# amansanghvi/Thesis

Measured on AMD Instinct MI355X. Metric: particle-updates/sec (particles x scans/s) @1081 beams, higher is better.
Workload: dtype int8 map cells (lattice log-odds), f64 poses/weights; 1 GPU; BASELINE configs[2]: room16 synthetic, 4096 particles/GPU, 1081 beams, 0.05 m grid, K=30 samples, both matcher stages, resample every step; particles_per_gpu=4096, beams=1081, parallelism=particles sharded x1

## Files before the change

thesis_amd/csrc/kernels_resample.hip:

```cpp
#include <limits.h>

#include "rbpf_internal.h"

namespace rbpf {

static const int PLAN_THREADS = 1024;

__device__ __forceinline__ dd dd_two_prod(double a, double b) {
    double p = a * b;
    double e = __fma_rn(a, b, -p);
    return {p, e};
}
__device__ __forceinline__ dd dd_mul_d(dd a, double b) {
    dd p = dd_two_prod(a.hi, b);
    double lo = p.lo + a.lo * b;
    double hi = p.hi + lo;
    return {hi, lo - (hi - p.hi)};
}
__device__ __forceinline__ dd dd_sub(dd a, dd b) { return dd_add(a, dd{-b.hi, -b.lo}); }
__device__ __forceinline__ dd dd_div_d(dd a, double b) {
    double q1 = a.hi / b;
    dd r = dd_sub(a, dd_two_prod(q1, b));
    double q2 = (r.hi + r.lo) / b;
    double hi = q1 + q2;
// ... 359 lines not shown
    if (threadIdx.x == 0) *n_pending = 0;
}

__global__ void export_weights_kernel(int P, const double* __restrict__ w, const int32_t* __restrict__ gid,
                                      double* __restrict__ out, int n_global, const uint8_t* __restrict__ bad) {
    int p = blockIdx.x * blockDim.x + threadIdx.x;
    if (p < P && gid[p] >= 0 && gid[p] < n_global) out[gid[p]] = w[p];
    if (p < P && bad && bad[p]) out[n_global] = 1.0;
}

__device__ void sources_to_T_stage(int P, const int32_t* __restrict__ idx, int32_t* __restrict__ T, int32_t* __restrict__ did) {
    __shared__ int s_buf[PLAN_THREADS];
    const int tid = threadIdx.x, nt = PLAN_THREADS;
    const int chunk = (P + nt - 1) / nt;
    const int i0 = min(tid * chunk, P), i1 = min(i0 + chunk, P);
    for (int i = i0; i < i1; ++i) T[i] = 0;
    __syncthreads();
    for (int j = i0; j < i1; ++j) if (idx[j] >= 0) atomicAdd(&T[idx[j]], 1);
    __syncthreads();
    int sum = 0;
    for (int i = i0; i < i1; ++i) sum += T[i];
    int total;
    int run = block_exclusive_scan_1024(sum, s_buf, tid, total);
    for (int i = i0; i < i1; ++i) { run += T[i]; T[i] = run; }
    if (tid == 0) *did = 1;
}

__global__ void gather_meta_kernel(DevView v, const int32_t* __restrict__ local_idx, int n, int32_t* __restrict__ out) {
    const int LL = v.L * v.L;
    int q = blockIdx.x * blockDim.x + threadIdx.x;
    if (q >= n * LL) return;
    const int i = q / LL, pos = q % LL;
    const int t = v.tile_tab[(size_t)v.slot[local_idx[i]] * LL + pos];
    int32_t* o = out + (size_t)q * 5;
    o[0] = t;
    for (int k = 0; k < 4; ++k) o[1 + k] = t >= 0 ? v.tile_bbox[4 * t + k] : 0;
}

struct PackJob { int32_t particle, tile, x0, x1, ya, yb; long long off; };

__global__ __launch_bounds__(BLOCK) void pack_kernel(DevView v, const PackJob* __restrict__ jobs, unsigned char* __restrict__ buf) {
    const PackJob j = jobs[blockIdx.x];
    const int tid = threadIdx.x;
    unsigned char* dst = buf + j.off;
    if (j.tile < 0) {
        if (tid < 13) {
            const int p = j.particle;
            double val = tid == 0 ? v.px[p] : tid == 1 ? v.py[p] : tid == 2 ? v.pth[p]
                       : tid < 12 ? v.cov[(size_t)(tid - 3) * v.P + p] : v.weight[p];
            reinterpret_cast<double*>(dst)[tid] = val;
        }
        return;
    }
    const size_t cells = (size_t)v.dim * v.dim;
    const int8_t* src = v.pool + (size_t)j.tile * cells;
    const int per_row = (j.yb - j.ya) / 16, rows = j.x1 - j.x0 + 1;
    for (int q = tid; q < rows * per_row; q += BLOCK) {
        const int x = j.x0 + q / per_row, y = j.ya + (q % per_row) * 16;
        reinterpret_cast<uint4*>(dst)[q] = *reinterpret_cast<const uint4*>(src + (size_t)x * v.dim + y);
    }
    uint32_t* docc = reinterpret_cast<uint32_t*>(dst + (size_t)rows * per_row * 16);
    const uint32_t* socc = v.occ + ((size_t)j.tile * v.dim + j.x0) * v.ow;
    for (int q = tid; q < rows * v.ow; q += BLOCK) docc[q] = socc[q];
}

struct UnpackJob { int32_t particle, pos, has, x0, x1, ya, yb, pad; long long off; };

__global__ __launch_bounds__(BLOCK) void unpack_kernel(DevView v, const UnpackJob* __restrict__ jobs, const unsigned char* __restrict__ buf,
                                                       int32_t* pending_free, int32_t* n_pending) {
    __shared__ int s_tile;
    const UnpackJob j = jobs[blockIdx.x];
    const int tid = threadIdx.x, LL = v.L * v.L;
    if (j.pos < 0) {
        if (tid < 13) {
            const double val = reinterpret_cast<const double*>(buf + j.off)[tid];
            const int p = j.particle;
            if (tid == 0) v.px[p] = val; else if (tid == 1) v.py[p] = val; else if (tid == 2) v.pth[p] = val;
            else if (tid < 12) v.cov[(size_t)(tid - 3) * v.P + p] = val; else v.weight[p] = 1.0;
        }
        return;
    }
    const int slot = v.slot[j.particle];
    int td = v.tile_tab[(size_t)slot * LL + j.pos];
    const size_t cells = (size_t)v.dim * v.dim;
    if (!j.has) {
        if (td < 0) return;
        int db[4];
        for (int k = 0; k < 4; ++k) db[k] = v.tile_bbox[4 * td + k];
        if (db[0] <= db[1] && db[2] <= db[3]) {
            copy_rows<BLOCK>(v.pool + (size_t)td * cells, nullptr, v.dim, db[0], db[1], db[2], db[3], tid);
            copy_occ_rows<BLOCK>(v.occ + (size_t)td * v.dim * v.ow, nullptr, v.ow, db[0], db[1], db[2], db[3], tid);
        }
        if (tid == 0) {
            v.tile_bbox[4 * td + 0] = INT_MAX; v.tile_bbox[4 * td + 1] = -1; v.tile_bbox[4 * td + 2] = INT_MAX; v.tile_bbox[4 * td + 3] = -1;
            v.tile_tab[(size_t)slot * LL + j.pos] = -1;
            pending_free[atomicAdd(n_pending, 1)] = td;
        }
        return;
    }
    if (td < 0) {
        if (tid == 0) {
            int idx = atomicSub(v.free_top, 1) - 1;
            if (idx < 0) { atomicAdd(v.free_top, 1); atomicCAS(v.err, 0, RBPF_ENOMEM); s_tile = -1; }
            else { s_tile = v.free_stack[idx]; v.tile_tab[(size_t)slot * LL + j.pos] = s_tile; }
        }
        __syncthreads();
        td = s_tile;
        if (td < 0) return;
    } else {
        int db[4];
        for (int k = 0; k < 4; ++k) db[k] = v.tile_bbox[4 * td + k];
        if (db[0] <= db[1] && db[2] <= db[3]) {
            copy_rows<BLOCK>(v.pool + (size_t)td * cells, nullptr, v.dim, db[0], db[1], db[2], db[3], tid);
            copy_occ_rows<BLOCK>(v.occ + (size_t)td * v.dim * v.ow, nullptr, v.ow, db[0], db[1], db[2], db[3], tid);
        }
        __syncthreads();
    }
    if (j.x0 <= j.x1) {
        const unsigned char* src = buf + j.off;
        int8_t* dst = v.pool + (size_t)td * cells;
        const int per_row = (j.yb - j.ya) / 16, rows = j.x1 - j.x0 + 1;
        for (int q = tid; q < rows * per_row; q += BLOCK) {
            const int x = j.x0 + q / per_row, y = j.ya + (q % per_row) * 16;
            *reinterpret_cast<uint4*>(dst + (size_t)x * v.dim + y) = reinterpret_cast<const uint4*>(src)[q];
        }
        const uint32_t* socc = reinterpret_cast<const uint32_t*>(src + (size_t)rows * per_row * 16);
        uint32_t* docc = v.occ + ((size_t)td * v.dim + j.x0) * v.ow;
        for (int q = tid; q < rows * v.ow; q += BLOCK) docc[q] = socc[q];
    }
    if (tid == 0) { v.tile_bbox[4 * td + 0] = j.x0; v.tile_bbox[4 * td + 1] = j.x1; v.tile_bbox[4 * td + 2] = j.ya; v.tile_bbox[4 * td + 3] = j.yb - 1; }
}

__global__ __launch_bounds__(PLAN_THREADS) void resample_plan_kernel(ResampleArgs a, PhaseArgs ph) {
    if (ph.phase == 1 ? !plan_phase_verdict(a.P, ph) : plan_phase_idle(ph)) return;
    resample_plan_stage(a);
}
__global__ void resample_expand_kernel(int P, const int32_t* __restrict__ T, int32_t* __restrict__ idx, PhaseArgs ph) {
    if (plan_phase_idle(ph)) return;
    const int j = blockIdx.x * blockDim.x + threadIdx.x;
    if (j < P) resample_expand_one(P, T, idx, j);
}
__global__ __launch_bounds__(PLAN_THREADS) void resample_pair_kernel(PairArgs a, PhaseArgs ph) {
    if (plan_phase_idle(ph)) {
        if (ph.phase == 1) plan_keep_stage(a.P, a.T, false, ph);
        return;
    }
    resample_pair_stage(a);
    if (ph.phase == 1) { __syncthreads(); plan_keep_stage(a.P, a.T, ph.leave_out && *a.did, ph); }
}
__global__ __launch_bounds__(PLAN_THREADS) void sources_to_T_kernel(int P, const int32_t* __restrict__ idx, int32_t* __restrict__ T,
                                                                     int32_t* __restrict__ did) { sources_to_T_stage(P, idx, T, did); }

enum { RS_PLAN = 1, RS_SRC2T = 2, RS_EXPAND = 4, RS_PAIR = 8, RS_GATHER = 16 };
static const int RS_FUSE_MAX = 4096;
static const int RS_GATHER_FUSE_MAX = 1024;
struct FusedArgs { int stages; ResampleArgs ra; int32_t* idx; PairArgs pa; GatherArgs ga; PhaseArgs ph; };
__global__ __launch_bounds__(PLAN_THREADS) void resample_fused_kernel(FusedArgs f) {
    extern __shared__ __align__(16) int32_t s_dyn[];
    int32_t* const s_T = s_dyn; int32_t* const s_idx = s_dyn + RS_FUSE_MAX;
    const int tid = threadIdx.x, P = f.ra.P;
#ifdef RBPF_STAMPS
    long long st[6]; st[0] = clock64();
#define RSTAMP(k) st[k] = clock64()
#else
#define RSTAMP(k) do { } while (0)
#endif
    if (f.ph.phase == 1) {
        if (!plan_phase_verdict(P, f.ph)) { plan_keep_stage(P, f.ra.T, false, f.ph); return; }
    } else if (plan_phase_idle(f.ph)) return;
    if (f.stages & RS_PLAN) { resample_plan_stage(f.ra); __syncthreads(); }
    RSTAMP(1);
    if (f.stages & RS_SRC2T) { sources_to_T_stage(P, f.idx, f.ra.T, f.ra.did); __syncthreads(); }
    for (int j = tid; j < P; j += PLAN_THREADS) s_T[j] = f.ra.T[j];
    __syncthreads();
    if (f.stages & RS_EXPAND) { for (int j = tid; j < P; j += PLAN_THREADS) { resample_expand_one(P, s_T, s_idx, j); f.idx[j] = s_idx[j]; } }
    else for (int j = tid; j < P; j += PLAN_THREADS) s_idx[j] = f.idx[j];
    __syncthreads();
    RSTAMP(2);
    if (f.stages & RS_PAIR) { PairArgs pa = f.pa; pa.T = s_T; pa.idx = s_idx; resample_pair_stage(pa); __syncthreads(); }
    if (f.ph.phase == 1) plan_keep_stage(P, s_T, f.ph.leave_out && *f.ra.did, f.ph);
    RSTAMP(3);
    if (f.stages & RS_GATHER) { GatherArgs ga = f.ga; ga.T = s_T; ga.idx = s_idx; for (int j = tid; j < ga.P; j += PLAN_THREADS) resample_gather_one(ga, j); }
    RSTAMP(4);
#ifdef RBPF_STAMPS
    if (tid == 0) printf("resample_fused: plan %lld expand %lld pair %lld gather %lld cycles\n", st[1] - st[0], st[2] - st[1], st[3] - st[2], st[4] - st[3]);
#endif
}

static void launch_resample_fused(const FusedArgs& f, hipStream_t s) {
    const size_t lds = 2 * RS_FUSE_MAX * sizeof(int32_t);
    static size_t lds_set[MAX_DEVICES] = {};
    ensure_dynamic_lds(reinterpret_cast<const void*>(resample_fused_kernel), lds, lds_set);
    hipLaunchKernelGGL(resample_fused_kernel, dim3(1), dim3(PLAN_THREADS), lds, s, f);
}

void launch_export_weights(const DevView& v, double* d_out, int n_global, const uint8_t* d_bad, hipStream_t s) {
    (void)hipMemsetAsync(d_out, 0, (size_t)(n_global + (d_bad ? 1 : 0)) * 8, s);
    hipLaunchKernelGGL(export_weights_kernel, dim3((v.P + 255) / 256), dim3(256), 0, s, v.P, v.weight, v.global_id, d_out, n_global, d_bad);
}
void launch_gather_meta(const DevView& v, const int32_t* d_local, int n, int32_t* d_out, hipStream_t s) {
    int tot = n * v.L * v.L;
    hipLaunchKernelGGL(gather_meta_kernel, dim3((tot + 255) / 256), dim3(256), 0, s, v, d_local, n, d_out);
}
void launch_pack(const DevView& v, const void* d_jobs, int n_jobs, void* d_buf, hipStream_t s) {
    if (n_jobs) hipLaunchKernelGGL(pack_kernel, dim3(n_jobs), dim3(BLOCK), 0, s, v, static_cast<const PackJob*>(d_jobs), static_cast<unsigned char*>(d_buf));
}
void launch_unpack(const DevView& v, const ResampleBuffers& b, const void* d_jobs, int n_jobs, const void* d_buf, hipStream_t s) {
    if (n_jobs) hipLaunchKernelGGL(unpack_kernel, dim3(n_jobs), dim3(BLOCK), 0, s, v, static_cast<const UnpackJob*>(d_jobs),
                                   static_cast<const unsigned char*>(d_buf), b.pending_free, b.n_pending);
    hipLaunchKernelGGL(resample_release_kernel, dim3(1), dim3(256), 0, s, v, b.pending_free, b.n_pending);
}

void launch_resample_indices(int P, const double* d_w, double u, double spread, int32_t* d_T, int32_t* d_idx,
                             int32_t* d_did, int32_t* d_err, hipStream_t s) {
    ResampleArgs ra{P, d_w, u, spread, d_T, d_did, d_err};
    if (P <= RS_FUSE_MAX) {
        FusedArgs f{RS_PLAN | RS_EXPAND, ra, d_idx, PairArgs{}, GatherArgs{}, PhaseArgs{}};
        launch_resample_fused(f, s);
        return;
    }
    hipLaunchKernelGGL(resample_plan_kernel, dim3(1), dim3(PLAN_THREADS), 0, s, ra, PhaseArgs{});
    hipLaunchKernelGGL(resample_expand_kernel, dim3((P + 255) / 256), dim3(256), 0, s, P, d_T, d_idx, PhaseArgs{});
}

static void launch_resample_planning(const DevView& v, const ResampleBuffers& b, const double* d_w, double u, double spread,
                                     const PhaseArgs& ph, hipStream_t s) {
    const PairArgs pa{v.P, b.T, b.idx, b.did, v.slot, b.slot2, b.dead_list, b.jobs, b.n_jobs, v.err};
    const GatherArgs ga{v.P, b.idx, b.did, v.px, v.py, v.pth, v.cov, v.weight, b.px2, b.py2, b.pth2, b.cov2, b.w2, b.T, v.dup_of};
    if (v.P > RS_FUSE_MAX) {
        if (d_w) {
            hipLaunchKernelGGL(resample_plan_kernel, dim3(1), dim3(PLAN_THREADS), 0, s, ResampleArgs{v.P, d_w, u, spread, b.T, b.did, v.err}, ph);
            hipLaunchKernelGGL(resample_expand_kernel, dim3((v.P + 255) / 256), dim3(256), 0, s, v.P, b.T, b.idx, ph);
        } else hipLaunchKernelGGL(sources_to_T_kernel, dim3(1), dim3(PLAN_THREADS), 0, s, v.P, b.idx, b.T, b.did);
        hipLaunchKernelGGL(resample_pair_kernel, dim3(1), dim3(PLAN_THREADS), 0, s, pa, ph);
    } else {
        FusedArgs f{(d_w ? RS_PLAN | RS_EXPAND : RS_SRC2T) | RS_PAIR | (v.P <= RS_GATHER_FUSE_MAX ? RS_GATHER : 0),
                    ResampleArgs{v.P, d_w, u, spread, b.T, b.did, v.err}, b.idx, pa, ga, ph};
        launch_resample_fused(f, s);
    }
}

void launch_resample_plan_early(const DevView& v, const ResampleBuffers& b, const uint8_t* d_bad, int leave_out, double u, double spread, hipStream_t s) {
    launch_resample_planning(v, b, v.weight, u, spread, PhaseArgs{1, d_bad, b.plan, b.skip, b.keep, leave_out, v.stats}, s);
}
void launch_resample_plan_late(const DevView& v, const ResampleBuffers& b, double u, double spread, hipStream_t s) {
    launch_resample_planning(v, b, v.weight, u, spread, PhaseArgs{2, nullptr, b.plan, b.skip, b.keep, 0, v.stats}, s);
}

void launch_resample_copies(const DevView& v, const ResampleBuffers& b, hipStream_t s) {
    const GatherArgs ga{v.P, b.idx, b.did, v.px, v.py, v.pth, v.cov, v.weight, b.px2, b.py2, b.pth2, b.cov2, b.w2, b.T, v.dup_of};
    CopyArgs ca{v, b.jobs, b.n_jobs, b.pending_free, b.n_pending, v.P <= RS_GATHER_FUSE_MAX ? 0 : 1, ga};
    hipLaunchKernelGGL(resample_copy_kernel, dim3(512), dim3(COPY_BLOCK), 0, s, ca);
    hipLaunchKernelGGL(resample_release_kernel, dim3(1), dim3(256), 0, s, v, b.pending_free, b.n_pending);
}

void launch_resample_local(const DevView& v, const ResampleBuffers& b, const double* d_w, double u, double spread, hipStream_t s) {
    launch_resample_planning(v, b, d_w, u, spread, PhaseArgs{}, s);
    launch_resample_copies(v, b, s);
}

}
```

thesis_amd/csrc/rbpf_api.hip:

```cpp
#include <math.h>
#include <stdio.h>
#include <stdlib.h>
#include <string.h>

#include <algorithm>
#include <initializer_list>
#include <limits>

#include "rbpf_host.h"
#include "rbpf_scanbatch.h"

using namespace rbpf;

static thread_local std::string g_create_err;

#define HIP_TRY(h, call)                                                                           \
    do {                                                                                           \
        hipError_t e_ = (call);                                                                    \
        if (e_ != hipSuccess) {                                                                    \
            (h)->err = std::string(#call) + ": " + hipGetErrorString(e_);                          \
            return RBPF_EDEVICE;                                                                   \
        }                                                                                          \
    } while (0)

// ... 140 lines not shown
        return fail(nullptr, RBPF_EINVAL, "log-odds constants have the wrong sign");
    cc.thr = (int)floor(c.occupied_threshold / c.quantum + 1e-9);

    int n_dev = 0;
    hipError_t e = hipGetDeviceCount(&n_dev);
    if (e == hipSuccess && (c.device < 0 || c.device >= n_dev)) e = hipErrorInvalidDevice;
    if (e != hipSuccess) { (void)hipGetLastError(); return fail(nullptr, RBPF_EDEVICE, std::string("device ") + std::to_string(c.device) + ": " + hipGetErrorString(e) +
                                     " (librbpf_hip needs an MI355X; there is no CPU path)"); }
    DevGuard dev_guard_(c.device);

    rbpf_handle* h = new rbpf_handle();
    h->cfg = c;
    memset(&h->counters, 0, sizeof(h->counters));
    DevView& v = h->v;
    memset(&v, 0, sizeof(v));
    v.P = c.n_particles; v.K = c.n_samples; v.B = 0; v.dim = dim; v.R = c.lattice_radius; v.L = 2 * v.R + 1;
    v.pool_tiles = c.pool_tiles > 0 ? c.pool_tiles : 2 * c.n_particles;
    if (v.pool_tiles < v.P) { delete h; return fail(nullptr, RBPF_EINVAL, "pool_tiles must be >= n_particles"); }
    v.cs = c.cell_size; v.tile_len = (double)c.tile_len_m;
    v.quantum = c.quantum;
    double inv = 1.0 / c.quantum;
    v.inv_quantum = fabs(inv - round(inv)) < 1e-9 ? round(inv) : 0.0;
    v.cc = cc;
    v.w_min_range = c.weight_min_range; v.w_max_range = c.weight_max_range;
    v.reach = (int)(c.max_ray_m / c.cell_size) + 3;

    {
        const int half = v.R * dim + dim / 2 + 2;
        std::vector<uint32_t>& lut = h->h_lut;
        int g_first = INT32_MAX;
        for (int g = -half; g <= half; ++g) {
            double pos = (double)g * v.cs;
            int lat;
            if (!tile_of_coord(pos, v.tile_len, v.R, lat)) { if (g_first != INT32_MAX) break; else continue; }
            double rel = pos - (double)lat * v.tile_len;
            int cidx = trunc_to_int(rel / v.cs + (double)dim / 2.0);
            if (cidx < 0 || cidx >= dim) { delete h; return fail(nullptr, RBPF_EINVAL, "cell index formula leaves the tile for this cell_size (the reference would raise IndexError)"); }
            if (g_first == INT32_MAX) g_first = g;
            uint32_t ent = ((uint32_t)(lat + v.R) << 16) | (uint32_t)cidx;
            if (!lut.empty() && ent < lut.back()) { delete h; return fail(nullptr, RBPF_EINVAL, "cell index formula is not monotone for this cell_size"); }
            lut.push_back(ent);
        }
        v.g_min = g_first; v.n_lut = (int)lut.size();
    }

    int rc = RBPF_OK;
    auto build = [&]() -> int {
        HIP_TRY(h, hipStreamCreateWithFlags(&h->stream, hipStreamNonBlocking));
        h->own_stream = true;
        for (int k = 0; k < rbpf_handle::N_KERN; ++k)
            for (int e = 0; e < 2; ++e) {
                h->ring[k][e].resize(rbpf_handle::RING);
                for (auto& ev : h->ring[k][e]) HIP_TRY(h, h->events.create(&ev, hipEventDisableSystemFence));
                h->begin_used[k].assign(rbpf_handle::RING, nullptr);
            }
        for (int e = 0; e < 2; ++e) {
            h->rs_mid[e].resize(rbpf_handle::RING);
            for (auto& ev : h->rs_mid[e]) HIP_TRY(h, h->events.create(&ev, hipEventDisableSystemFence));
        }
        h->rs_split.assign(rbpf_handle::RING, 0);
        const size_t P = v.P, LL = (size_t)v.L * v.L, cells = (size_t)dim * dim;
        uint32_t* d_lut; ALLOC(h, d_lut, h->h_lut.size()); v.lut = d_lut;
        HIP_TRY(h, hipMemcpy(d_lut, h->h_lut.data(), h->h_lut.size() * 4, hipMemcpyHostToDevice));
        {
            const int KW = (dim + WIN - 1) / WIN;
            std::vector<int32_t> gw((size_t)v.L * (KW + 1));
            for (int a = 0; a < v.L; ++a)
                for (int k = 0; k <= KW; ++k) {
                    uint32_t key = k < KW ? (((uint32_t)a << 16) | (uint32_t)(k * WIN)) : ((uint32_t)(a + 1) << 16);
                    auto it = std::lower_bound(h->h_lut.begin(), h->h_lut.end(), key);
                    gw[(size_t)a * (KW + 1) + k] = v.g_min + (int32_t)(it - h->h_lut.begin());
                }
            int32_t* d_gw; ALLOC(h, d_gw, gw.size()); v.gwin = d_gw;
            HIP_TRY(h, hipMemcpy(d_gw, gw.data(), gw.size() * 4, hipMemcpyHostToDevice));
        }
        ALLOC(h, v.px, P); ALLOC(h, v.py, P); ALLOC(h, v.pth, P); ALLOC(h, v.cov, 9 * P); ALLOC(h, v.weight, P);
        ALLOC(h, v.slot, P); ALLOC(h, v.global_id, P);
        v.ow = (dim + 31) / 32;
        ALLOC(h, v.tile_tab, P * LL); ALLOC(h, v.pool, (size_t)v.pool_tiles * cells);
        ALLOC(h, v.occ, (size_t)v.pool_tiles * dim * v.ow + 4);
        HIP_TRY(h, hipMemset(v.occ, 0, (size_t)v.pool_tiles * dim * v.ow * 4));
        ALLOC(h, v.tile_bbox, (size_t)v.pool_tiles * 4); ALLOC(h, v.free_stack, v.pool_tiles); ALLOC(h, v.free_top, 1);
        {
            const size_t MB = (size_t)c.max_beams, MBP = (MB + 15) & ~(size_t)15;
            const size_t MBW = (MB + 63) & ~(size_t)63;
            h->scan_bytes = 3 * MBP * 8 + 4 * MBP * 4 + MBP + 2 * MBW * 4 + MBW * 2;
            ALLOC(h, h->d_scan, h->scan_bytes);
            unsigned char* d = h->d_scan;
            v.bx = reinterpret_cast<double*>(d); v.by = v.bx + MBP; v.bscale = v.by + MBP;
            v.msel_x = reinterpret_cast<float*>(d + 3 * MBP * 8); v.msel_y = v.msel_x + MBP; v.asel_x = v.msel_y + MBP; v.asel_y = v.asel_x + MBP;
            v.bflags = d + 3 * MBP * 8 + 4 * MBP * 4;
            v.wsel_x = reinterpret_cast<const float*>(d + 3 * MBP * 8 + 4 * MBP * 4 + MBP); v.wsel_y = v.wsel_x + MBW;
            v.wsel_idx = reinterpret_cast<const uint16_t*>(v.wsel_y + MBW);
            HIP_TRY(h, h->rings[R_SCAN].create(h->scan_bytes));
            HIP_TRY(h, h->rings[R_LAST].create(MB * 16));
            HIP_TRY(h, h->rings[R_IDX].create((size_t)P * 8));
        }
        ALLOC(h, v.upd_pose, 3 * P);
        ALLOC(h, v.prop_prep, 24 * P);
        ALLOC(h, v.prop_samp, 256 * P);
        ALLOC(h, v.stats, ST_COUNT); ALLOC(h, v.err, 1);
        ALLOC(h, v.mu_fallback, P); HIP_TRY(h, hipMemset(v.mu_fallback, 0, P * 4));
        ALLOC(h, v.ev_queue, 2); HIP_TRY(h, hipMemset(v.ev_queue, 0, 8));
        ALLOC(h, h->d_did_early, 1);
        HIP_TRY(h, hipMemset(h->d_did_early, 0, 4));
        HIP_TRY(h, h->events.create(&h->ev_weights, hipEventDisableTiming | hipEventDisableSystemFence));
        {
            v.mu_mode = env_is("RBPF_MAP_KERNEL", "window") ? MU_WINDOW : env_is("RBPF_MAP_KERNEL", "ray") ? MU_RAY : env_is("RBPF_MAP_KERNEL", "ev") ? MU_EV : MU_DEFAULT;
            v.ev_resident = env_is("RBPF_EV_RESIDENT", "0") ? 0 : 1;
            const char* eg = getenv("RBPF_EV_GRID");
            v.ev_grid = eg ? std::max(0, atoi(eg)) : 0;
            v.match_stage_slow = env_is("RBPF_MATCH_STAGE", "slow") ? 1 : 0;
            const char* ws = getenv("RBPF_WSAFE");
            v.wsafe_override = ws ? (float)atof(ws) : -1.0f;
            v.weight_entry_f64 = env_is("RBPF_WEIGHT_ENTRY", "f64") ? 1 : 0;
            v.ndt_refine = h->cfg.ndt_refine;
            h->dedup_enabled = !env_is("RBPF_MATCH_DEDUP", "0");
            {
                int cus = 0;
                if (hipDeviceGetAttribute(&cus, hipDeviceAttributeMultiprocessorCount, c.device) != hipSuccess || cus < 1) { (void)hipGetLastError(); cus = 1; }
                h->skip_discarded = !env_is("RBPF_SKIP_DISCARDED", "0");
                h->hold_back = getenv("RBPF_SKIP_DISCARDED") ? true : (long long)P > 4LL * cus;
                const bool halves = env_is("RBPF_SCAN_HALVES", "0") ? false : getenv("RBPF_SCAN_HALVES") ? true : ((long long)P >= SCAN_HALVES_MIN_PER_CU * cus && (long long)P < SCAN_HALVES_END_PER_CU * cus);
                if (halves) {
                    int least = 0, greatest = 0;
                    HIP_TRY(h, hipDeviceGetStreamPriorityRange(&least, &greatest));
                    HIP_TRY(h, hipStreamCreateWithPriority(&h->side, hipStreamNonBlocking, greatest));
                    HIP_TRY(h, h->events.create(&h->ev_fork, hipEventDisableTiming | hipEventDisableSystemFence));
                    HIP_TRY(h, h->events.create(&h->ev_half_match, hipEventDisableSystemFence));
                    HIP_TRY(h, h->events.create(&h->ev_half_weight, hipEventDisableSystemFence));
                    h->halves_first = (int)(P - std::max<size_t>(P > 1 ? 1 : 0, 3 * P / 8));
                }
            }
        }
        ALLOC(h, v.dup_of, P); v.dups_valid = 0;
        ALLOC(h, h->d_last_xy, 2 * (size_t)c.max_beams); ALLOC(h, h->d_tmp_sel, 2 * (size_t)c.max_beams);
        if (raycast_lds_bytes(c.max_beams, v.reach) > LDS_LIMIT) return fail(h, RBPF_EINVAL, "max_beams too large for the LDS window layout");
        match_geometry(c, c.cell_size, h->mN, h->mds, h->mmcs, h->md0, h->mncr);
        h->mlds = match_lds_bytes(h->mN, c.max_beams, match_max_coarse(h->mncr, 0.7, h->mmcs), match_per_rot(0.7, h->mmcs));
        if (h->mlds > LDS_LIMIT) return fail(h, RBPF_EINVAL, "matcher region does not fit in LDS for this cell_size");
        if (c.ndt_refine && ndt_cells(h->mmcs) >= 2) {
            if (ndt_lds_bytes(h->mN, c.max_beams) > LDS_LIMIT) return fail(h, RBPF_EINVAL, "NDT stage: matcher region does not fit in LDS");
            ALLOC(h, v.ndt_occ, P * (size_t)h->mN * (h->mN / 32)); ALLOC(h, v.ndt_aux, 5 * P);
        }
        ALLOC(h, h->d_match, 13 * P); ALLOC(h, h->d_bad, P); ALLOC(h, h->d_guess_full, P * (size_t)c.n_samples * 3);
        {
            ResampleBuffers& r = h->rs;
            ALLOC(h, r.T, P); ALLOC(h, r.idx, P); ALLOC(h, r.did, 1); ALLOC(h, r.slot2, P); ALLOC(h, r.dead_list, P);
            ALLOC(h, r.jobs, 2 * P); ALLOC(h, r.n_jobs, 2); ALLOC(h, r.pending_free, (size_t)v.pool_tiles); ALLOC(h, r.n_pending, 1);
            ALLOC(h, r.px2, P); ALLOC(h, r.py2, P); ALLOC(h, r.pth2, P); ALLOC(h, r.cov2, 9 * P); ALLOC(h, r.w2, P);
            ALLOC(h, r.skip, P); ALLOC(h, r.keep, P); ALLOC(h, r.plan, 2);
            HIP_TRY(h, hipMemset(r.n_pending, 0, 4)); HIP_TRY(h, hipMemset(r.n_jobs, 0, 8)); HIP_TRY(h, hipMemset(r.did, 0, 4));
            HIP_TRY(h, hipMemset(r.skip, 0, P)); HIP_TRY(h, hipMemset(r.plan, 0, 8));
        }
        HIP_TRY(h, hipMemset(v.pool, 0, (size_t)v.pool_tiles * cells));
        HIP_TRY(h, hipMemset(v.px, 0, P * 8)); HIP_TRY(h, hipMemset(v.py, 0, P * 8)); HIP_TRY(h, hipMemset(v.pth, 0, P * 8));
        HIP_TRY(h, hipMemset(v.cov, 0, 9 * P * 8));
        HIP_TRY(h, hipMemset(v.stats, 0, ST_COUNT * 8)); HIP_TRY(h, hipMemset(v.err, 0, 4));
        std::vector<double> w(P, 1.0);
        HIP_TRY(h, hipMemcpy(v.weight, w.data(), P * 8, hipMemcpyHostToDevice));
        std::vector<int32_t> ids(P), tab(P * LL, -1), fs(v.pool_tiles), bb((size_t)v.pool_tiles * 4);
        for (size_t p = 0; p < P; ++p) { ids[p] = (int32_t)p; tab[p * LL + (size_t)v.R * v.L + v.R] = (int32_t)p; }
        for (int t = 0; t < v.pool_tiles; ++t) { bb[4 * t] = INT32_MAX; bb[4 * t + 1] = -1; bb[4 * t + 2] = INT32_MAX; bb[4 * t + 3] = -1; }
        int32_t top = v.pool_tiles - (int32_t)P;
        for (int i = 0; i < top; ++i) fs[i] = v.pool_tiles - 1 - i;
        HIP_TRY(h, hipMemcpy(v.slot, ids.data(), P * 4, hipMemcpyHostToDevice));
        HIP_TRY(h, hipMemcpy(v.global_id, ids.data(), P * 4, hipMemcpyHostToDevice));
        HIP_TRY(h, hipMemcpy(v.tile_tab, tab.data(), P * LL * 4, hipMemcpyHostToDevice));
        HIP_TRY(h, hipMemcpy(v.free_stack, fs.data(), (size_t)v.pool_tiles * 4, hipMemcpyHostToDevice));
        HIP_TRY(h, hipMemcpy(v.free_top, &top, 4, hipMemcpyHostToDevice));
        HIP_TRY(h, hipMemcpy(v.tile_bbox, bb.data(), bb.size() * 4, hipMemcpyHostToDevice));
        return RBPF_OK;
    };
    rc = build();
    if (rc != RBPF_OK) { g_create_err = h->err; rbpf_destroy(h); return rc; }
    *out = h;
    return RBPF_OK;
}

int rbpf_destroy(rbpf_handle* h) {
    if (!h) return RBPF_OK;
    ON_DEVICE_HELD(h);
    h->mu_pending = false;
    if (hipStreamSynchronize(h->stream) != hipSuccess) (void)hipGetLastError();
    if (h->side && hipStreamSynchronize(h->side) != hipSuccess) (void)hipGetLastError();
    h->each_staging([](Staging& s) { if (s.wait() != hipSuccess) (void)hipGetLastError(); });
    if (h->ev_weights_valid && hipEventSynchronize(h->ev_weights) != hipSuccess) (void)hipGetLastError();
    for (Block& b : h->allocs) b.release();
    for (Block& b : h->buf) b.release();
    for (Block& b : h->track_mem) b.release();
    h->each_staging([](Staging& s) { s.release(); });
    h->each_staging([](Staging& s) { s.destroy_event(); });
    h->events.destroy();
    if (h->own_stream && h->stream) (void)hipStreamDestroy(h->stream);
    if (h->side) (void)hipStreamDestroy(h->side);
    (void)hipGetLastError();
    delete h;
    return RBPF_OK;
}

const char* rbpf_last_error(const rbpf_handle* h) { return h ? h->err.c_str() : g_create_err.c_str(); }

int rbpf_set_stream(rbpf_handle* h, void* s) {
    if (!h) return RBPF_EINVAL;
    ON_DEVICE(h);
    HIP_TRY(h, hipStreamSynchronize(h->stream));
    if (h->own_stream && h->stream) (void)hipStreamDestroy(h->stream);
    h->own_stream = false;
    h->stream = static_cast<hipStream_t>(s);
    h->last_end = nullptr;
    return RBPF_OK;
}

int rbpf_release_stream(rbpf_handle* h) {
    if (!h) return RBPF_EINVAL;
    ON_DEVICE(h);
    if (h->own_stream) return RBPF_OK;
    HIP_TRY(h, hipStreamSynchronize(h->stream));
    if (h->early_n > 0) HIP_TRY(h, h->stage[S_EARLY].wait());
    h->stream = nullptr;
    HIP_TRY(h, hipStreamCreateWithFlags(&h->stream, hipStreamNonBlocking));
    h->own_stream = true;
    h->last_end = nullptr;
    return RBPF_OK;
}

int rbpf_abi_struct_bytes(int32_t* config_bytes, int32_t* counters_bytes) {
    if (config_bytes) *config_bytes = (int32_t)sizeof(rbpf_config);
    if (counters_bytes) *counters_bytes = (int32_t)sizeof(rbpf_counters);
    return RBPF_OK;
}

int rbpf_synchronize(rbpf_handle* h) {
    if (!h) return RBPF_EINVAL;
    ON_DEVICE(h);
    return check_device_error(h);
}

int rbpf_set_profiling_families(rbpf_handle* h, uint32_t mask) {
    if (!h) return RBPF_EINVAL;
    ON_DEVICE(h);
    return rbpf_set_profiling(h, mask ? (int)(0x100u | (mask & 0x1Fu)) : 0);
}

int rbpf_set_profiling(rbpf_handle* h, int on) {
    if (!h) return RBPF_EINVAL;
    ON_DEVICE(h);
    h->profiling = on != 0;
    h->prof_mask = !on ? 0u : (on & 0x100) ? ((unsigned)on & 0x1Fu) : 0x1Fu;
    for (int k = 0; k < rbpf_handle::N_KERN; ++k) h->ring_n[k] = 0;
    h->last_end = nullptr;
    HIP_TRY(h, hipMemsetAsync(h->v.stats, 0, ST_COUNT * sizeof(unsigned long long), h->stream));
    return RBPF_OK;
}

int rbpf_get_kernel_ms(rbpf_handle* h, int32_t which, double* out_ms, int32_t cap, int32_t* n_out) {
    if (!h || !n_out || which < 0 || which >= rbpf_handle::N_KERN) return RBPF_EINVAL;
    ON_DEVICE(h);
    HIP_TRY(h, hipStreamSynchronize(h->stream));
    int n = std::min(h->ring_n[which], rbpf_handle::RING);
    int first = h->ring_n[which] - n;
    int m = 0;
    for (int i = 0; i < n && m < cap; ++i) {
        int slot = (first + i) % rbpf_handle::RING;
        float ms = 0;
        if (h->family_ms(which, slot, &ms) != hipSuccess) { (void)hipGetLastError(); continue; }
        if (out_ms) out_ms[m] = ms;
        ++m;
    }
    *n_out = m;
    return RBPF_OK;
}

int rbpf_get_counters(rbpf_handle* h, rbpf_counters* out) {
    if (!h || !out) return RBPF_EINVAL;
    ON_DEVICE(h);
    unsigned long long st[ST_COUNT];
    int32_t top = 0;
    HIP_TRY(h, hipMemcpyAsync(st, h->v.stats, sizeof(st), hipMemcpyDeviceToHost, h->stream));
    HIP_TRY(h, hipMemcpyAsync(&top, h->v.free_top, 4, hipMemcpyDeviceToHost, h->stream));
    HIP_TRY(h, hipStreamSynchronize(h->stream));
    rbpf_counters& c = h->counters;
    c.scan_updates = h->scan_updates;
    c.ray_cells_visited = st[ST_RAY_CELLS]; c.cells_written = st[ST_CELLS_WRITTEN];
    c.cells_gathered = st[ST_GATHERS]; c.slow_cells = st[ST_SLOW_CELLS];
    c.resample_copies = st[ST_COPIES]; c.bytes_copied = st[ST_COPY_BYTES];
    c.tiles_in_use = (uint64_t)(h->v.pool_tiles - top);
    c.window_fallbacks = st[ST_WINDOW_FALLBACKS];
    c.ndt_runs = st[ST_NDT_RUNS]; c.ndt_evaluations = st[ST_NDT_EVALS]; c.ndt_accepted = st[ST_NDT_ACCEPTED];
    c.match_shared = st[ST_MATCH_SHARED];
    for (int k = 0; k < 7; ++k) c.reserved[k] = st[8 + k];
    c.stamp7 = st[15];
    {
        auto sat16 = [](unsigned long long x) { return x > 65535ull ? 65535ull : x; };
        c.fallback_reasons = sat16(st[ST_FALLBACK_REASONS]) | (sat16(st[ST_FB_BOUND]) << 16) | (sat16(st[ST_FB_TABLES]) << 32);
        c.fallback_geometry = st[ST_FALLBACK_REASONS]; c.fallback_bound = st[ST_FB_BOUND]; c.fallback_tables = st[ST_FB_TABLES];
        c.map_events = st[ST_MAP_EVENTS]; c.map_event_overflows = st[ST_EV_OVERFLOWS];
    }
    c.map_windows = st[ST_MAP_WINDOWS];
    c.map_updates_skipped = st[ST_MU_SKIPPED];
    c.map_pool_cells = st[ST_POOL_CELLS]; c.map_near_cells = st[ST_NEAR_CELLS];
    if (h->profiling) {
        double* dst[5] = {&c.ms_raycast, &c.ms_weight, &c.ms_resample, &c.ms_match, &c.ms_ndt};
        for (int k = 0; k < 5; ++k) {
            if (h->ring_n[k] == 0) continue;
            int slot = (h->ring_n[k] - 1) % rbpf_handle::RING;
// ... 2436 lines not shown
```

thesis_amd/csrc/rbpf_internal.h:

```cpp
#pragma once
#include <hip/hip_runtime.h>
#include <stdint.h>
#include <mutex>

#include "../../include/rbpf_hip.h"
#include "rbpf_math.h"
#include "rbpf_blockrelax.h"

namespace rbpf {

static const int MAX_DEVICES = 16;
inline void ensure_dynamic_lds(const void* fn, size_t bytes, size_t* set) {
    static std::mutex mu;
    std::lock_guard<std::mutex> lock(mu);
    int dev = 0;
    (void)hipGetDevice(&dev);
    const bool tracked = dev >= 0 && dev < MAX_DEVICES;
    if (tracked && bytes <= set[dev]) return;
    const hipError_t rc = hipFuncSetAttribute(fn, hipFuncAttributeMaxDynamicSharedMemorySize, (int)bytes);
    if (rc != hipSuccess) { (void)hipGetLastError(); return; }
    if (tracked) set[dev] = bytes;
}


static const int BLOCK = 256;
static const int WIN = 128;
static const int MAX_ITEMS_PER_PARTICLE = 64;

enum { BF_WEIGHT = 1, BF_MATCH = 2, BF_LONG = 4, BF_MATCH_ADJ = 8 };

enum MapKernelMode : int {
    MU_DEFAULT,
    MU_WINDOW,
    MU_RAY,
    MU_EV,
};

struct DevView {
    int P, K, B, dim, R, L;
    int pool_tiles;
    int reach;
    double cs, tile_len;
    double quantum, inv_quantum;
    CellConsts cc;
    double w_min_range, w_max_range;
    const uint32_t* lut; int g_min, n_lut;
    const int32_t* gwin;
    double *px, *py, *pth;
    double *cov;
    double *weight;
    int32_t* slot;
    int32_t* global_id;
    int32_t* tile_tab;
    int8_t*  pool;
    uint32_t* occ;
    int ow;
    int32_t* tile_bbox;
    int32_t* free_stack;
    int32_t* free_top;
    const double *bx, *by, *bscale;
    const uint8_t* bflags;
    float *msel_x, *msel_y; int n_msel;
    float *asel_x, *asel_y; int n_asel;
    const float *wsel_x, *wsel_y; const uint16_t* wsel_idx; int n_wsel;
    double*  upd_pose;
    double*  prop_prep;
    double*  prop_samp;
    int32_t* mu_fallback;
    MapKernelMode mu_mode;
    const uint8_t* mu_skip;
    const int32_t* mu_keep;
    const int32_t* mu_n_keep;
    uint32_t* ev_queue;
    int ev_resident, ev_grid;
    uint32_t* ndt_occ; double* ndt_aux;
    int ndt_refine;
    int32_t* dup_of; int dups_valid;
    float wsafe_override;
    int weight_entry_f64;
    int match_stage_slow;
    unsigned long long* stats;
    int32_t* err;
};

struct ResampleBuffers {
    int32_t *T, *idx, *did;
    int32_t *slot2, *dead_list, *jobs;
    int32_t *n_jobs;
    int32_t *pending_free, *n_pending;
    double *px2, *py2, *pth2, *cov2, *w2;
    uint8_t* skip; int32_t* keep;
    int32_t* plan;
};

enum { ST_RAY_CELLS = 0, ST_CELLS_WRITTEN = 1, ST_GATHERS = 2, ST_SLOW_CELLS = 3,
       ST_COPIES = 4, ST_COPY_BYTES = 5, ST_WINDOW_FALLBACKS = 6, ST_FALLBACK_REASONS = 7,
       ST_NDT_RUNS = 16, ST_NDT_EVALS = 17, ST_NDT_ACCEPTED = 18, ST_MATCH_SHARED = 19, ST_MAP_WINDOWS = 20,
       ST_FB_BOUND = 21, ST_FB_TABLES = 22, ST_MAP_EVENTS = 23, ST_EV_OVERFLOWS = 24, ST_MU_SKIPPED = 25,
       ST_POOL_CELLS = 26, ST_NEAR_CELLS = 27, ST_COUNT = 28 };

struct RenderJob {
    int32_t pos;
    int32_t i0, j0;
    int32_t ni, jlo, jhi;
    int32_t ox, oy;
};
struct RenderFilter {
    const RenderJob* jobs;
    const double* lut;
    const double* w;
    double S;
    int C, ngroups;
    long long ny;
    size_t ncell;
    float *prob, *occ;
    double *part_p, *part_o;
};
struct LoadTile { int32_t pos, i0, i1, j0, j1; };
struct LoadArgs {
    const RenderJob* jobs;
    const LoadTile* tiles; int n_tiles;
    const int8_t* cells;
    long long ny, ncell;
    int p_lo, p_hi;
    int32_t* bad;
};
struct PlaceArgs {
    const int8_t* src;
    int nsx, nsy;
    double c, s, ox, oy;
    double src_cell, cs;
    int S, mode;
    int x0, y0;
    long long ny, ncell;
    int8_t* warped; uint8_t* covered;
    const int32_t* bad;
};
struct CastArgs {
    const double* pose4;
    const double* beam2;
    int n_poses, B;
    int particle;
    double inv, tlim, max_range;
    double* ranges; uint8_t* status;
};
struct GainArgs {
    const double* pose4;
    const double* beam2;
    const int32_t* table;
    int n_poses, B, nv;
    int particle;
    int M, W;
    double inv, tlim;
    int64_t* gain; int32_t *seen, *unknown;
};
struct BuildArgs {
    const double* pose4;
    const double* beam2;
    const double* ranges;
    uint32_t* ends;
    int n_scans, B;
    int M, W;
    int x0, y0, nx, ny;
    double inv, tlim;
    double min_range, max_range;
    int32_t *hits, *seen;
};
static const int REFINE_BLOCK = 512;
static const int REFINE_RUN = 8;
static const int REFINE_TABLE = 2048;
__host__ __device__ inline int refine_runs(int nw, int s) { return ((((nw + (1 << s) - 1) >> s) + REFINE_RUN - 1) / REFINE_RUN) << s; }
struct RefineArgs {
    int N, B;
    int Wt, R, s, nk, kpw;
    int Mw, WW;
    int fx0, fy0, frows, fW;
    double invS, min_range, max_range;
    const double* guess;
    const int32_t* cell0;
    const double* rot;
    const double* beam2;
    const double* ranges;
    const uint2* field;
    unsigned long long* packed;
    int32_t *guess_score, *n_used;
    int32_t* scores;
    double* out_pose; int32_t* out_n6;
};
static const int PAIRS_BLOCK = 512;
struct PairsArgs {
    int M, B;
    int Mw, WW;
    double inv, min_range, max_range;
    const double* pose4;
    const double* beam2;
    const double* ranges;
    const int32_t* query;
    const int32_t* runs;
    const int32_t* cell0;
    uint2* fields;
    int32_t* n_ref;
    double* out_pose; int32_t* out_m8;
};
struct PlacesArgs {
    int nq, nr, R, k;
    int chunk, nch;
    const unsigned long long* qd;
    const unsigned long long* rd;
    const int32_t* limit;
    unsigned long long* dil;
    int32_t* w;
    int4* partial;
    int32_t *out_qk4, *out_q2;
};
static const int SURFACE_BLOCK = 512;
static const int SURFACE_MAX_PEAKS = 8;
static const int SURFACE_SUMS = 11;
struct SurfaceArgs {
    int N, R, W;
    int ex_t, ex_r, K;
    const int32_t* scores;
    const int32_t* drop;
    long long* out;
    int32_t* count;
};
struct LocateArgs {
    int particle;
    int x0, y0, nx, ny;
    int nyw;
    int M;
    int rows, W;
    int n_rot, nb, rpw;
    double inv;
    const double* cs;
    const double* bxy;
    int32_t* offs;
    uint2* field;
    uint32_t* cand;
    int32_t* items; int32_t* n_items;
    uint32_t* packed;
    int32_t *best, *rot;
};
struct AlignArgs {
    int x0, y0, nx, ny;
    int nyw;
    int M;
// ... 178 lines not shown
```

Before: 2.405 million particle-updates/s.

## Rewrite fused resample kernel with register-chunked scans and 16-bit LDS

Rewrites the single-block fused resample kernel so each thread owns a contiguous chunk of particles in registers. Planning (a double-double prefix sum), expansion (binary search over T), pairing (dead/dup compaction through one packed block scan) and keep-list construction now run inline instead of calling the separate stage helpers. LDS arrays shrink to uint16, which lets the fused path cover up to 16384 particles, with template specialisations for chunk sizes 1, 4 and 16. The intent is fewer serial passes and barriers inside the one-block resample critical path. The cost is code duplication, a dependence on 16-bit index storage, and an environment-variable cap on the fused size.

New measurement: 2.412 million particle-updates/s, median of 6. No clear change (+0.3%).

```diff
diff --git a/thesis_amd/csrc/kernels_resample.hip b/thesis_amd/csrc/kernels_resample.hip
--- a/thesis_amd/csrc/kernels_resample.hip
+++ b/thesis_amd/csrc/kernels_resample.hip
@@ -535,35 +535,238 @@
                                                                      int32_t* __restrict__ did) { sources_to_T_stage(P, idx, T, did); }
 
 enum { RS_PLAN = 1, RS_SRC2T = 2, RS_EXPAND = 4, RS_PAIR = 8, RS_GATHER = 16 };
-static const int RS_FUSE_MAX = 4096;
+static const int RS_INDICES_FUSE_MAX = 4096;
 static const int RS_GATHER_FUSE_MAX = 1024;
+static const int RS_WAVES = PLAN_THREADS / 64;
 struct FusedArgs { int stages; ResampleArgs ra; int32_t* idx; PairArgs pa; GatherArgs ga; PhaseArgs ph; };
+
+__device__ __forceinline__ unsigned long long block_exclusive_scan_u64(unsigned long long val, unsigned long long* s_buf, int tid,
+                                                                      unsigned long long& all) {
+    const int lane = tid & 63, wave = tid >> 6;
+    unsigned long long incl = val;
+    for (int off = 1; off < 64; off <<= 1) { const unsigned long long n = __shfl_up(incl, off, 64); if (lane >= off) incl += n; }
+    __syncthreads();
+    if (lane == 63) s_buf[wave] = incl;
+    __syncthreads();
+    unsigned long long base = 0, tot = 0;
+    for (int q = 0; q < RS_WAVES; ++q) { const unsigned long long x = s_buf[q]; if (q < wave) base += x; tot += x; }
+    all = tot;
+    return base + incl - val;
+}
+
+template <int CH>
 __global__ __launch_bounds__(PLAN_THREADS) void resample_fused_kernel(FusedArgs f) {
-    extern __shared__ __align__(16) int32_t s_dyn[];
-    int32_t* const s_T = s_dyn; int32_t* const s_idx = s_dyn + RS_FUSE_MAX;
-    const int tid = threadIdx.x, P = f.ra.P;
+    extern __shared__ __align__(16) uint16_t s_dyn[];
+    const int tid = threadIdx.x, lane = tid & 63, wave = tid >> 6, P = f.ra.P;
+    const int n16 = (P + 7) & ~7;
+    uint16_t* const s_T = s_dyn; uint16_t* const s_idx = s_dyn + n16;
+    uint16_t* const s_dead = s_dyn + 2 * n16; uint16_t* const s_slot = s_dyn + 3 * n16;
+    __shared__ double s_red[3 * RS_WAVES];
+    __shared__ double s_whi[RS_WAVES], s_wlo[RS_WAVES];
+    __shared__ double s_bhi[RS_WAVES + 1], s_blo[RS_WAVES + 1];
+    __shared__ unsigned long long s_scan[RS_WAVES];
+    const bool plan = f.stages & RS_PLAN, src2t = f.stages & RS_SRC2T, pair = f.stages & RS_PAIR;
+    const int chunk = (P + PLAN_THREADS - 1) / PLAN_THREADS;
+    const int i0 = min(tid * chunk, P), cnt = min(i0 + chunk, P) - i0;
 #ifdef RBPF_STAMPS
     long long st[6]; st[0] = clock64();
 #define RSTAMP(k) st[k] = clock64()
 #else
 #define RSTAMP(k) do { } while (0)
 #endif
+    double w[CH]; int t[CH], ix[CH];
+    int any_bad = 0;
+#pragma unroll
+    for (int k = 0; k < CH; ++k) {
+        w[k] = 0.0; t[k] = 0; ix[k] = -1;
+        if (k < cnt) {
+            const int i = i0 + k;
+            if (plan) w[k] = f.ra.w[i];
+            if (src2t) ix[k] = f.idx[i];
+            if (pair) s_slot[i] = (uint16_t)f.pa.slot_old[i];
+            if (f.ph.phase == 1) any_bad |= f.ph.bad[i];
+        }
+    }
+    const int standing = f.ph.phase == 2 ? f.ph.plan[1] : 0;
     if (f.ph.phase == 1) {
-        if (!plan_phase_verdict(P, f.ph)) { plan_keep_stage(P, f.ra.T, false, f.ph); return; }
-    } else if (plan_phase_idle(f.ph)) return;
-    if (f.stages & RS_PLAN) { resample_plan_stage(f.ra); __syncthreads(); }
+        any_bad = __syncthreads_or(any_bad);
+        if (tid == 0) f.ph.plan[1] = any_bad ? 0 : 1;
+        if (any_bad) {
+#pragma unroll
+            for (int k = 0; k < CH; ++k) if (k < cnt) { f.ph.skip[i0 + k] = 0; f.ph.keep[i0 + k] = i0 + k; }
+            if (tid == 0) f.ph.plan[0] = P;
+            return;
+        }
+    } else if (standing != 0) return;
+    int did = 1;
+    if (plan) {
+        double mx = -INFINITY, mn = INFINITY, mn2 = INFINITY;
+#pragma unroll
+        for (int k = 0; k < CH; ++k) if (k < cnt) {
+            mx = fmax(mx, w[k]); mn = fmin(mn, w[k]); mn2 = fmin(mn2, w[k] == -INFINITY ? 0.0 : w[k]);
+        }
+        for (int o = 32; o > 0; o >>= 1) {
+            mx = fmax(mx, __shfl_xor(mx, o, 64)); mn = fmin(mn, __shfl_xor(mn, o, 64)); mn2 = fmin(mn2, __shfl_xor(mn2, o, 64));
+        }
+        if (lane == 0) { s_red[wave] = mx; s_red[RS_WAVES + wave] = mn; s_red[2 * RS_WAVES + wave] = mn2; }
+        __syncthreads();
+        mx = s_red[lane & (RS_WAVES - 1)]; mn = s_red[RS_WAVES + (lane & (RS_WAVES - 1))]; mn2 = s_red[2 * RS_WAVES + (lane & (RS_WAVES - 1))];
+        for (int o = RS_WAVES / 2; o > 0; o >>= 1) {
+            mx = fmax(mx, __shfl_xor(mx, o, 64)); mn = fmin(mn, __shfl_xor(mn, o, 64)); mn2 = fmin(mn2, __shfl_xor(mn2, o, 64));
+        }
+        if (!((mx - mn) > f.ra.spread)) {
+            did = 0;
+#pragma unroll
+            for (int k = 0; k < CH; ++k) t[k] = i0 + k + 1;
+        } else {
+            const double shift = mn2 < 0 ? fabs(mn2) : 0.0;
+            auto adj = [&](double x) -> dd {
+                if (x == -INFINITY) return dd{0.0, 0.0};
+                if (shift != 0.0 && x != 0.0) return dd_two_sum(x, shift);
+                return dd{x, 0.0};
+            };
+            dd tot = {0.0, 0.0};
+#pragma unroll
+            for (int k = 0; k < CH; ++k) if (k < cnt) tot = dd_add(tot, adj(w[k]));
+            dd incl = tot;
+            for (int off = 1; off < 64; off <<= 1) {
+                const dd n = {__shfl_up(incl.hi, off, 64), __shfl_up(incl.lo, off, 64)};
+                if (lane >= off) incl = dd_add(n, incl);
+            }
+            if (lane == 63) { s_whi[wave] = incl.hi; s_wlo[wave] = incl.lo; }
+            __syncthreads();
+            if (wave == 0) {
+                dd r = {0.0, 0.0};
+                for (int q = 0; q < RS_WAVES; ++q) {
+                    if (lane == 0) { s_bhi[q] = r.hi; s_blo[q] = r.lo; }
+                    r = dd_add(r, dd{s_whi[q], s_wlo[q]});
+                }
+                if (lane == 0) { s_bhi[RS_WAVES] = r.hi; s_blo[RS_WAVES] = r.lo; }
+            }
+            __syncthreads();
+            const dd wbase = {s_bhi[wave], s_blo[wave]}, total = {s_bhi[RS_WAVES], s_blo[RS_WAVES]};
+            dd prev = {__shfl_up(incl.hi, 1, 64), __shfl_up(incl.lo, 1, 64)};
+            if (lane == 0) prev = dd{0.0, 0.0};
+            dd run = dd_add(wbase, prev);
+            const dd slice = dd_div_d(total, (double)P);
+            const dd start = dd_mul_d(slice, f.ra.u);
+            const bool bad = !(slice.hi > 0) || !isfinite(slice.hi);
+#pragma unroll
+            for (int k = 0; k < CH; ++k) if (k < cnt) {
+                run = dd_add(run, adj(w[k]));
+                long long tt = bad ? 0 : dd_floor_div(dd_sub(run, start), slice) + 1;
+                if (tt < 0) tt = 0;
+                if (tt > P) tt = (long long)P + 1;
+                t[k] = (int)tt;
+                if (i0 + k == P - 1 && t[k] != P) atomicCAS(f.ra.err, 0, RBPF_ESTATE);
+            }
+        }
+        if (tid == 0) *f.ra.did = did;
+    } else {
+        int32_t* const s_cnt = reinterpret_cast<int32_t*>(s_dyn);
+#pragma unroll
+        for (int k = 0; k < CH; ++k) if (k < cnt) s_cnt[i0 + k] = 0;
+        __syncthreads();
+#pragma unroll
+        for (int k = 0; k < CH; ++k) if (k < cnt && (unsigned)ix[k] < (unsigned)P) atomicAdd(&s_cnt[ix[k]], 1);
+        __syncthreads();
+        int sum = 0;
+#pragma unroll
+        for (int k = 0; k < CH; ++k) if (k < cnt) { t[k] = s_cnt[i0 + k]; sum += t[k]; }
+        unsigned long long all;
+        int run = (int)block_exclusive_scan_u64((unsigned long long)sum, s_scan, tid, all);
+#pragma unroll
+        for (int k = 0; k < CH; ++k) if (k < cnt) { run += t[k]; t[k] = run; }
+        if (tid == 0) *f.ra.did = 1;
+    }
+#pragma unroll
+    for (int k = 0; k < CH; ++k) if (k < cnt) {
+        f.ra.T[i0 + k] = t[k]; s_T[i0 + k] = (uint16_t)t[k];
+        if (src2t) s_idx[i0 + k] = (uint16_t)ix[k];
+    }
+    __syncthreads();
     RSTAMP(1);
-    if (f.stages & RS_SRC2T) { sources_to_T_stage(P, f.idx, f.ra.T, f.ra.did); __syncthreads(); }
-    for (int j = tid; j < P; j += PLAN_THREADS) s_T[j] = f.ra.T[j];
-    __syncthreads();
-    if (f.stages & RS_EXPAND) { for (int j = tid; j < P; j += PLAN_THREADS) { resample_expand_one(P, s_T, s_idx, j); f.idx[j] = s_idx[j]; } }
-    else for (int j = tid; j < P; j += PLAN_THREADS) s_idx[j] = f.idx[j];
-    __syncthreads();
+    if (f.stages & RS_EXPAND) {
+        int hi[CH];
+#pragma unroll
+        for (int k = 0; k < CH; ++k) { ix[k] = 0; hi[k] = k < cnt ? P - 1 : 0; }
+        bool more;
+        do {
+            more = false;
+#pragma unroll
+            for (int k = 0; k < CH; ++k) if (ix[k] < hi[k]) {
+                const int mid = (ix[k] + hi[k]) >> 1;
+                if ((int)s_T[mid] > i0 + k) hi[k] = mid; else ix[k] = mid + 1;
+                more = true;
+            }
+        } while (more);
+#pragma unroll
+        for (int k = 0; k < CH; ++k) if (k < cnt) { f.idx[i0 + k] = ix[k]; s_idx[i0 + k] = (uint16_t)ix[k]; }
+        __syncthreads();
+    }
     RSTAMP(2);
-    if (f.stages & RS_PAIR) { PairArgs pa = f.pa; pa.T = s_T; pa.idx = s_idx; resample_pair_stage(pa); __syncthreads(); }
-    if (f.ph.phase == 1) plan_keep_stage(P, s_T, f.ph.leave_out && *f.ra.did, f.ph);
+    if (pair) {
+        unsigned dead = 0, dup = 0, in = 0;
+        int pt = i0 > 0 ? (int)s_T[i0 - 1] : 0, pi = i0 > 0 ? (int)(int16_t)s_idx[i0 - 1] : -1;
+#pragma unroll
+        for (int k = 0; k < CH; ++k) if (k < cnt) {
+            if (t[k] - pt == 0) dead |= 1u << k;
+            if (ix[k] < 0) in |= 1u << k; else if (i0 + k > 0 && ix[k] == pi) dup |= 1u << k;
+            pt = t[k]; pi = ix[k];
+        }
+        const int n_dead = __popc(dead), n_dup = __popc(dup | in), n_job = __popc(dup);
+        unsigned long long all;
+        const unsigned long long base = block_exclusive_scan_u64((unsigned long long)n_dead | (unsigned long long)n_dup << 20 |
+                                                                 (unsigned long long)n_job << 40, s_scan, tid, all);
+        const int dead_base = (int)(base & 0xFFFFF), total_dead = (int)(all & 0xFFFFF), total_dup = (int)(all >> 20 & 0xFFFFF);
+        int db = dead_base, dbase = (int)(base >> 20 & 0xFFFFF), jbase = (int)(base >> 40);
+#pragma unroll
+        for (int k = 0; k < CH; ++k) if (dead >> k & 1) s_dead[db++] = (uint16_t)(i0 + k);
+        __syncthreads();
+#pragma unroll
+        for (int k = 0; k < CH; ++k) if (k < cnt) {
+            if ((dup | in) >> k & 1) {
+                const int dst = s_slot[dbase < total_dead ? s_dead[dbase] : 0];
+                if (dup >> k & 1) { f.pa.jobs[2 * jbase] = s_slot[ix[k]]; f.pa.jobs[2 * jbase + 1] = dst; ++jbase; }
+                f.pa.slot_new[i0 + k] = dst;
+                ++dbase;
+            } else {
+                f.pa.slot_new[i0 + k] = s_slot[ix[k]];
+            }
+        }
+        if (tid == 0) {
+            if (total_dup != total_dead) atomicCAS(f.pa.err, 0, RBPF_ESTATE);
+            f.pa.n_jobs[0] = (int)(all >> 40); f.pa.n_jobs[1] = 0;
+        }
+        if (f.ph.phase == 1) {
+            const bool leave = f.ph.leave_out && did;
+            int kb = leave ? i0 - dead_base : i0;
+#pragma unroll
+            for (int k = 0; k < CH; ++k) if (k < cnt) {
+                const bool out = leave && (dead >> k & 1);
+                f.ph.skip[i0 + k] = out ? 1 : 0;
+                if (!out) f.ph.keep[kb++] = i0 + k;
+            }
+            if (tid == 0) {
+                const int stay = leave ? P - total_dead : P;
+                f.ph.plan[0] = stay;
+                if (stay < P) atomicAdd(&f.ph.stats[ST_MU_SKIPPED], (unsigned long long)(P - stay));
+            }
+        }
+    }
     RSTAMP(3);
-    if (f.stages & RS_GATHER) { GatherArgs ga = f.ga; ga.T = s_T; ga.idx = s_idx; for (int j = tid; j < ga.P; j += PLAN_THREADS) resample_gather_one(ga, j); }
+    if (f.stages & RS_GATHER) {
+        const GatherArgs& a = f.ga;
+        for (int j = tid; j < P; j += PLAN_THREADS) {
+            const int i = (int16_t)s_idx[j];
+            if (a.dup_of) a.dup_of[j] = (i >= 0 && did) ? (i > 0 ? (int)s_T[i - 1] : 0) : j;
+            if (i < 0) continue;
+            a.px2[j] = a.px[i]; a.py2[j] = a.py[i]; a.pth2[j] = a.pth[i];
+#pragma unroll
+            for (int k = 0; k < 9; ++k) a.cov2[(size_t)k * P + j] = a.cov[(size_t)k * P + i];
+            a.w2[j] = did ? 1.0 : a.w[i];
+        }
+    }
     RSTAMP(4);
 #ifdef RBPF_STAMPS
     if (tid == 0) printf("resample_fused: plan %lld expand %lld pair %lld gather %lld cycles\n", st[1] - st[0], st[2] - st[1], st[3] - st[2], st[4] - st[3]);
@@ -571,10 +774,20 @@
 }
 
 static void launch_resample_fused(const FusedArgs& f, hipStream_t s) {
-    const size_t lds = 2 * RS_FUSE_MAX * sizeof(int32_t);
-    static size_t lds_set[MAX_DEVICES] = {};
-    ensure_dynamic_lds(reinterpret_cast<const void*>(resample_fused_kernel), lds, lds_set);
-    hipLaunchKernelGGL(resample_fused_kernel, dim3(1), dim3(PLAN_THREADS), lds, s, f);
+    const int P = f.ra.P;
+    const size_t lds = (size_t)4 * ((P + 7) & ~7) * sizeof(uint16_t);
+    const size_t lds_max = (size_t)4 * RS_FUSE_MAX * sizeof(uint16_t);
+    static size_t lds_set[3][MAX_DEVICES] = {};
+    if (P <= PLAN_THREADS) {
+        ensure_dynamic_lds(reinterpret_cast<const void*>(resample_fused_kernel<1>), lds_max / 16, lds_set[0]);
+        hipLaunchKernelGGL(resample_fused_kernel<1>, dim3(1), dim3(PLAN_THREADS), lds, s, f);
+    } else if (P <= 4 * PLAN_THREADS) {
+        ensure_dynamic_lds(reinterpret_cast<const void*>(resample_fused_kernel<4>), lds_max / 4, lds_set[1]);
+        hipLaunchKernelGGL(resample_fused_kernel<4>, dim3(1), dim3(PLAN_THREADS), lds, s, f);
+    } else {
+        ensure_dynamic_lds(reinterpret_cast<const void*>(resample_fused_kernel<16>), lds_max, lds_set[2]);
+        hipLaunchKernelGGL(resample_fused_kernel<16>, dim3(1), dim3(PLAN_THREADS), lds, s, f);
+    }
 }
 
 void launch_export_weights(const DevView& v, double* d_out, int n_global, const uint8_t* d_bad, hipStream_t s) {
@@ -597,7 +810,7 @@
 void launch_resample_indices(int P, const double* d_w, double u, double spread, int32_t* d_T, int32_t* d_idx,
                              int32_t* d_did, int32_t* d_err, hipStream_t s) {
     ResampleArgs ra{P, d_w, u, spread, d_T, d_did, d_err};
-    if (P <= RS_FUSE_MAX) {
+    if (P <= RS_INDICES_FUSE_MAX) {
         FusedArgs f{RS_PLAN | RS_EXPAND, ra, d_idx, PairArgs{}, GatherArgs{}, PhaseArgs{}};
         launch_resample_fused(f, s);
         return;
@@ -605,19 +818,21 @@
     hipLaunchKernelGGL(resample_plan_kernel, dim3(1), dim3(PLAN_THREADS), 0, s, ra, PhaseArgs{});
     hipLaunchKernelGGL(resample_expand_kernel, dim3((P + 255) / 256), dim3(256), 0, s, P, d_T, d_idx, PhaseArgs{});
 }
+
+static bool gather_fused(const DevView& v, const ResampleBuffers& b) { return v.P <= RS_GATHER_FUSE_MAX && v.P <= b.fuse_max; }
 
 static void launch_resample_planning(const DevView& v, const ResampleBuffers& b, const double* d_w, double u, double spread,
                                      const PhaseArgs& ph, hipStream_t s) {
     const PairArgs pa{v.P, b.T, b.idx, b.did, v.slot, b.slot2, b.dead_list, b.jobs, b.n_jobs, v.err};
     const GatherArgs ga{v.P, b.idx, b.did, v.px, v.py, v.pth, v.cov, v.weight, b.px2, b.py2, b.pth2, b.cov2, b.w2, b.T, v.dup_of};
-    if (v.P > RS_FUSE_MAX) {
+    if (v.P > b.fuse_max) {
         if (d_w) {
             hipLaunchKernelGGL(resample_plan_kernel, dim3(1), dim3(PLAN_THREADS), 0, s, ResampleArgs{v.P, d_w, u, spread, b.T, b.did, v.err}, ph);
             hipLaunchKernelGGL(resample_expand_kernel, dim3((v.P + 255) / 256), dim3(256), 0, s, v.P, b.T, b.idx, ph);
         } else hipLaunchKernelGGL(sources_to_T_kernel, dim3(1), dim3(PLAN_THREADS), 0, s, v.P, b.idx, b.T, b.did);
         hipLaunchKernelGGL(resample_pair_kernel, dim3(1), dim3(PLAN_THREADS), 0, s, pa, ph);
     } else {
-        FusedArgs f{(d_w ? RS_PLAN | RS_EXPAND : RS_SRC2T) | RS_PAIR | (v.P <= RS_GATHER_FUSE_MAX ? RS_GATHER : 0),
+        FusedArgs f{(d_w ? RS_PLAN | RS_EXPAND : RS_SRC2T) | RS_PAIR | (gather_fused(v, b) ? RS_GATHER : 0),
                     ResampleArgs{v.P, d_w, u, spread, b.T, b.did, v.err}, b.idx, pa, ga, ph};
         launch_resample_fused(f, s);
     }
@@ -632,7 +847,7 @@
 
 void launch_resample_copies(const DevView& v, const ResampleBuffers& b, hipStream_t s) {
     const GatherArgs ga{v.P, b.idx, b.did, v.px, v.py, v.pth, v.cov, v.weight, b.px2, b.py2, b.pth2, b.cov2, b.w2, b.T, v.dup_of};
-    CopyArgs ca{v, b.jobs, b.n_jobs, b.pending_free, b.n_pending, v.P <= RS_GATHER_FUSE_MAX ? 0 : 1, ga};
+    CopyArgs ca{v, b.jobs, b.n_jobs, b.pending_free, b.n_pending, gather_fused(v, b) ? 0 : 1, ga};
     hipLaunchKernelGGL(resample_copy_kernel, dim3(512), dim3(COPY_BLOCK), 0, s, ca);
     hipLaunchKernelGGL(resample_release_kernel, dim3(1), dim3(256), 0, s, v, b.pending_free, b.n_pending);
 }
diff --git a/thesis_amd/csrc/rbpf_api.hip b/thesis_amd/csrc/rbpf_api.hip
--- a/thesis_amd/csrc/rbpf_api.hip
+++ b/thesis_amd/csrc/rbpf_api.hip
@@ -316,6 +316,8 @@
             ALLOC(h, r.skip, P); ALLOC(h, r.keep, P); ALLOC(h, r.plan, 2);
             HIP_TRY(h, hipMemset(r.n_pending, 0, 4)); HIP_TRY(h, hipMemset(r.n_jobs, 0, 8)); HIP_TRY(h, hipMemset(r.did, 0, 4));
             HIP_TRY(h, hipMemset(r.skip, 0, P)); HIP_TRY(h, hipMemset(r.plan, 0, 8));
+            const char* fm = getenv("RBPF_RS_FUSE_MAX");
+            r.fuse_max = fm ? std::min(RS_FUSE_MAX, std::max(0, atoi(fm))) : RS_FUSE_MAX;
         }
         HIP_TRY(h, hipMemset(v.pool, 0, (size_t)v.pool_tiles * cells));
         HIP_TRY(h, hipMemset(v.px, 0, P * 8)); HIP_TRY(h, hipMemset(v.py, 0, P * 8)); HIP_TRY(h, hipMemset(v.pth, 0, P * 8));
diff --git a/thesis_amd/csrc/rbpf_internal.h b/thesis_amd/csrc/rbpf_internal.h
--- a/thesis_amd/csrc/rbpf_internal.h
+++ b/thesis_amd/csrc/rbpf_internal.h
@@ -91,7 +91,9 @@
     double *px2, *py2, *pth2, *cov2, *w2;
     uint8_t* skip; int32_t* keep;
     int32_t* plan;
-};
+    int fuse_max;
+};
+static const int RS_FUSE_MAX = 16384;
 
 enum { ST_RAY_CELLS = 0, ST_CELLS_WRITTEN = 1, ST_GATHERS = 2, ST_SLOW_CELLS = 3,
        ST_COPIES = 4, ST_COPY_BYTES = 5, ST_WINDOW_FALLBACKS = 6, ST_FALLBACK_REASONS = 7,
```
